# RobertKajnak/AMT-SAGA

Hardware: AMD Instinct MI355X
Metric: audio windows/sec (44.1 kHz, 2048-pt STFT) through full detect->subtract loop (higher is better)
Workload: dtype f32 (conv: split-fp16 x2 operands, f32 accumulate; 4x16 layers on the large images in the FFT domain); 1 GPU; C3: 1024 polyphonic piano windows, STFT(2048) + pitch+velocity+timing(start,end) heads + 1 subtraction iteration; windows_per_gpu=1024, n_fft=2048, hop=512, frames=516, iters=1, parallelism=windows sharded x1, event all-gather

## Files before the change

### amt-saga_amd/amt_saga/rdcnn.py

```python
import ctypes as C
import hashlib
import json
import os

import numpy as np
import torch

from . import _lib
from .device import empty, ptr, require_gpu, stream_ptr, to_dev


DEFAULT_MODE = int(os.environ.get('AMT_CONV_MODE', '3'))

_CALIBRATION_FILE = os.path.join(os.path.dirname(os.path.abspath(__file__)), 'data', 'synthetic_heads.npz')
_calibration = None


def topology_signature(cfg, seed):
    blob = json.dumps({k: cfg[k] for k in sorted(cfg)}, sort_keys=True, default=list)
    return '%s-s%d' % (hashlib.sha1(blob.encode()).hexdigest()[:10], int(seed))


def _calibration_table():
    global _calibration
# ... 204 lines not shown
        h = C.c_void_p()
        _lib.check(lib.amt_rdcnn_create(C.byref(h), C.byref(d),
                                        self._blob.ctypes.data_as(C.c_void_p), self._blob.size))
        self._net = h
        self._lib = lib
        _lib.check(lib.amt_rdcnn_set_mode(h, int(getattr(self, 'mode', DEFAULT_MODE))))

    def _release(self):
        if getattr(self, '_net', None) is not None:
            self._lib.amt_rdcnn_destroy(self._net)
        self._net = None
        self._ws = None
        if getattr(self, '_trainer', None) is not None:
            self._tlib.amt_trainer_destroy(self._trainer)
        self._trainer = None
        self._trained = False

    def __del__(self):
        try:
            self._release()
        except Exception:
            pass

    def load_weights(self, filename):
        with open(filename, 'rb') as fh:
            magic = fh.read(8)
        if magic == b'\x89HDF\r\n\x1a\n':
            from .keras_io import load_keras_weights
            self.set_weights(load_keras_weights(filename, self.layout))
            return
        with np.load(filename) as z:
            self.set_weights({k: z[k] for k in z.files})

    def save_weights(self, filename):
        self._sync_from_trainer()
        if str(filename).endswith(('.h5', '.hdf5')):
            from .keras_io import save_keras_weights
            save_keras_weights(filename, self.weights, self.cfg)
        else:
            np.savez(filename, **self.weights)

    @property
    def flops_per_window(self):
        self._ensure()
        return float(self._lib.amt_rdcnn_flops_per_window(self._net))

    @property
    def fc_pooled_layers(self):
        self._ensure()
        fn = self._lib.amt_rdcnn_fc_pooled_layers
        fn.restype, fn.argtypes = C.c_int, [C.c_void_p]
        return int(fn(self._net))

    PLAN_IMPLS = ('first_mfma', 'first_valu', 'fft_row', 'fft_packed', 'f16x3', 'bf16x6', 'f32')
    PLAN_KEYS = ('impl', 'kh', 'kw', 'cin', 'cout', 'H', 'W', 'cw', 'TH', 'TW', 'NWIN', 'masked', 'wm_ms', 'nslice', 'MT')

    def layer_plans(self, mode=None):
        self._ensure()
        fn = self._lib.amt_rdcnn_layer_plan
        fn.restype, fn.argtypes = C.c_int, [C.c_void_p, C.c_int, C.c_int, C.c_int, C.c_void_p]
        mode = self.mode if mode is None else int(mode)
        out = []
        for t in range(len(self.cfg['input_shapes'])):
            plans = []
            for i in range(self.cfg['convolutional_layer_count']):
                v = np.zeros(len(self.PLAN_KEYS), np.int32)
                _lib.check(fn(self._net, t, i, mode, v.ctypes.data_as(C.c_void_p)))
                p = dict(zip(self.PLAN_KEYS, map(int, v)), tower=t, layer=i + 1, mode=mode)
                p['impl'] = self.PLAN_IMPLS[p['impl']]
                plans.append(p)
            out.append(plans)
        return out

    def layer_outputs(self, xs):
        self._ensure()
        fn = self._lib.amt_rdcnn_layer_tap
        fn.restype, fn.argtypes = C.c_int, [C.c_void_p, C.c_int, C.c_int, C.c_void_p]
        B = xs[0].shape[0]
        acts = [[empty((B, p['H'], p['W'], p['cout'])) for p in plans] for plans in self.layer_plans()]
        try:
            for t, row in enumerate(acts):
                for i, a in enumerate(row):
                    _lib.check(fn(self._net, t, i, ptr(a)))
            y, lg = self.predict_device(xs, return_logits=True)
        finally:
            for t, row in enumerate(acts):
                for i in range(len(row)):
                    fn(self._net, t, i, None)
        return y, lg, acts

    def set_mode(self, mode):
        self.mode = int(mode)
        if self._net is not None:
            _lib.check(self._lib.amt_rdcnn_set_mode(self._net, self.mode))

    def profile(self, enable=True):
        self._ensure()
        _lib.check(self._lib.amt_rdcnn_profile(self._net, int(bool(enable))))

    def profile_read(self, reset=True):
        self._ensure()
        n = C.c_int32(0)
        _lib.check(self._lib.amt_rdcnn_profile_read(self._net, None, None, None, None, 0, C.byref(n), 0))
        cap = n.value
        desc = np.zeros((cap, 8), np.int32)
        ms = np.zeros(cap); win = np.zeros(cap); fl = np.zeros(cap)
# ... 150 lines not shown
```

### amt-saga_amd/csrc/amt_fftconv.h

```cpp
#pragma once
#include "amt_common.h"
#include "amt_launch.h"

struct amt_fftconv_layer;

struct FcEpilogue {
    const float *s1 = nullptr, *t1 = nullptr, *s2 = nullptr, *t2 = nullptr;
    const float *sc = nullptr; size_t sc_stride = 0;
    const float *sc1 = nullptr; size_t sc1_stride = 0;
    const float *sc1_w = nullptr, *sc1_s = nullptr, *sc1_t = nullptr;
    float *wmax = nullptr, *wavg = nullptr; size_t wp_stride = 0;
};

struct FcBnCopies {
    float *s1 = nullptr, *t1 = nullptr, *s2 = nullptr, *t2 = nullptr;
    hipError_t upload(const float *hs1, const float *ht1, const float *hs2, const float *ht2, int channels) {
        const float *h[4] = {hs1, ht1, hs2, ht2};
        float **d[4] = {&s1, &t1, &s2, &t2};
        hipError_t e = hipSuccess;
        for (int i = 0; i < 4 && e == hipSuccess; ++i) {
            if (h[i]) e = hipMalloc(d[i], channels * sizeof(float));
            if (h[i] && e == hipSuccess) e = hipMemcpy(*d[i], h[i], channels * sizeof(float), hipMemcpyHostToDevice);
        }
        return e;
    }
    void release() {
        for (float **p : {&s1, &t1, &s2, &t2}) { if (*p) (void)hipFree(*p); *p = nullptr; }
    }
};

int amt_fftconv_layer_create_internal(amt_fftconv_layer **out, const float *kernel);
void amt_fftconv_layer_destroy_internal(amt_fftconv_layer *L);
size_t amt_fftconv_freq_floats(int B, int H);
int amt_fftconv_forward_fft(const amt_fftconv_layer *L, const float *in_sp, size_t in_stride, int B, int H, int W,
                            float *Xf, float *amaxf, hipStream_t st);
int amt_fftconv_gemm(const amt_fftconv_layer *L, const float *Xf, const float *amaxf, int B, int H, float *Yf, hipStream_t st);
int amt_fftconv_inverse_epilogue(const amt_fftconv_layer *L, const float *Yf, const FcEpilogue &ep, int B, int H, int W,
                                 float *out_sp, size_t out_stride, float *Xf_next, float *amaxf_next, float *amax_out,
                                 hipStream_t st);

struct amt_fftpk_layer;
int amt_fftpk_layer_create_internal(amt_fftpk_layer **out, const float *kernel);
void amt_fftpk_layer_destroy_internal(amt_fftpk_layer *L);
size_t amt_fftpk_freq_floats(int B);
int amt_fftpk_forward_fft(const amt_fftpk_layer *L, const float *in_sp, size_t in_stride, int B, float *Xf, float *amaxf, hipStream_t st);
int amt_fftpk_gemm(const amt_fftpk_layer *L, const float *Xf, const float *amaxf, int B, float *Yf, hipStream_t st);
int amt_fftpk_inverse_epilogue(const amt_fftpk_layer *L, const float *Yf, const FcEpilogue &ep, int B, float *out_sp, size_t out_stride,
                               float *Xf_next, float *amaxf_next, float *amax_out, hipStream_t st);

struct FcLayer {
    amt_fftconv_layer *row = nullptr;
    amt_fftpk_layer *pk = nullptr;
    int H = 0, W = 0;
    explicit operator bool() const { return row || pk; }
};
static inline size_t fc_freq_floats(const FcLayer &l, int B) {
    return l.pk ? amt_fftpk_freq_floats(B) : amt_fftconv_freq_floats(B, l.H);
}
static inline int fc_forward_fft(const FcLayer &l, const float *in_sp, size_t in_stride, int B, float *Xf, float *amaxf, hipStream_t st) {
    return l.pk ? amt_fftpk_forward_fft(l.pk, in_sp, in_stride, B, Xf, amaxf, st)
                : amt_fftconv_forward_fft(l.row, in_sp, in_stride, B, l.H, l.W, Xf, amaxf, st);
}
static inline int fc_gemm(const FcLayer &l, const float *Xf, const float *amaxf, int B, float *Yf, hipStream_t st) {
    return l.pk ? amt_fftpk_gemm(l.pk, Xf, amaxf, B, Yf, st) : amt_fftconv_gemm(l.row, Xf, amaxf, B, l.H, Yf, st);
}
static inline int fc_inverse_epilogue(const FcLayer &l, const float *Yf, const FcEpilogue &ep, int B, float *out_sp, size_t out_stride,
                                      float *Xf_next, float *amaxf_next, float *amax_out, hipStream_t st) {
    return l.pk ? amt_fftpk_inverse_epilogue(l.pk, Yf, ep, B, out_sp, out_stride, Xf_next, amaxf_next, amax_out, st)
                : amt_fftconv_inverse_epilogue(l.row, Yf, ep, B, l.H, l.W, out_sp, out_stride, Xf_next, amaxf_next, amax_out, st);
}
```

### amt-saga_amd/csrc/amt_fftconv.hip

```cpp
#include "amt_fftconv_dev.h"
#include "amt_fftconv.h"
#include <algorithm>
#include <cmath>
#include <cstdlib>
#include <vector>

#define FC_NF 576
#define FC_NP 289
#define FC_PS 1158
#define FC_THREADS 384

struct FcRowArgs {
    const float *in_sp; size_t in_stride;
    const float *Yf;
    float *out_sp; size_t out_stride;
    float *Xf;
    float *amaxf;
    float *amax_out;
    const float *s1, *t1, *s2, *t2;
    const float *sc; size_t sc_stride;
    const float *sc1; size_t sc1_stride;
    const float *sc1_w, *sc1_s, *sc1_t;
    const float2 *tw;
    int B, H, W;
    int sf, sh;
    float *wmax, *wavg; size_t wp_stride;
};

template <bool IN_FREQ, int EPI>
__global__ __launch_bounds__(FC_THREADS, 4) void fc_row_kernel(FcRowArgs a) {
    extern __shared__ __attribute__((aligned(16))) float fc_smem[];
    const int tid = threadIdx.x;
    float *buf = fc_smem;
    float2 *tw = reinterpret_cast<float2 *>(fc_smem + 16 * FC_PS);
    const int c16 = (tid >> 2) & 15;
    const int j24 = (tid & 3) + 4 * (tid >> 6);
    const int row = blockIdx.x;
    const int b = row / a.H, h = row - b * a.H;
    for (int i = tid; i < FC_NF; i += FC_THREADS) tw[i] = a.tw[i];
    float2 x[24];
    if (IN_FREQ) {
        const int k1 = j24;
        const float *yb = a.Yf + (size_t)b * FC_NP * a.H * 64 + (size_t)h * a.sh;
        const unsigned int vlo = (unsigned)((k1 * a.sf + 2 * c16) * 4);
        const unsigned int vhi = (unsigned)(((FC_NF - k1) * a.sf + 32 + 2 * c16) * 4);
        const int kstep = 24 * a.sf;
#pragma unroll
        for (int k2 = 0; k2 < 24; ++k2) {
            if (k2 < 12) x[k2] = fc_at<float2>(yb + k2 * kstep, vlo);
            else if (k2 > 12) x[k2] = fc_at<float2>(yb - k2 * kstep, vhi);
            else x[k2] = fc_at<float2>(yb, k1 == 0 ? vlo + (unsigned)(12 * kstep * 4) : vhi - (unsigned)(12 * kstep * 4));
        }
        fc_fft24<true>(x);
        __syncthreads();
#pragma unroll
        for (int g0 = 0; g0 < 24; g0 += 8) {
            float2 w[8];
#pragma unroll
            for (int i = 0; i < 8; ++i) w[i] = tw[(g0 + i) * k1];
            __builtin_amdgcn_sched_barrier(0);
#pragma unroll
            for (int i = 0; i < 8; ++i) {
                const float2 v = fc_cmulc(x[g0 + i], w[i]);
                *reinterpret_cast<float2 *>(buf + c16 * FC_PS + ((g0 + i) * 24 + k1) * 2) = v;
            }
        }
        __syncthreads();
        const int n2 = j24;
#pragma unroll
        for (int k = 0; k < 24; ++k) x[k] = *reinterpret_cast<const float2 *>(buf + c16 * FC_PS + (n2 * 24 + k) * 2);
        fc_fft24<true>(x);
        const float inv_n = 1.0f / (float)FC_NF;
        int c0 = 2 * c16;
        if constexpr (EPI == 5) asm volatile("" : "+v"(c0));
        const float k1a = -a.s1[c0] * (inv_n * FC_LOG2E), k1b = -a.s1[c0 + 1] * (inv_n * FC_LOG2E);
        const float k0a = -a.t1[c0] * FC_LOG2E, k0b = -a.t1[c0 + 1] * FC_LOG2E;
        if constexpr (EPI == 1) {
#pragma unroll
            for (int n1 = 0; n1 < 24; ++n1) {
                float2 v;
                v.x = fc_sigmoid_affine(x[n1].x, k1a, k0a);
                v.y = fc_sigmoid_affine(x[n1].y, k1b, k0b);
                if (24 * n1 + n2 >= a.W) v = make_float2(0.f, 0.f);
                x[n1] = v;
            }
        } else {
            constexpr bool RES = EPI == 2 || EPI == 3 || EPI == 5;
            constexpr bool IDSC = EPI == 2 || EPI == 5;
            const float s2a = RES ? a.s2[c0] : 1.f, s2b = RES ? a.s2[c0 + 1] : 1.f;
            const float t2a = RES ? a.t2[c0] : 0.f, t2b = RES ? a.t2[c0 + 1] : 0.f;
            const float *scb = IDSC ? a.sc + (size_t)b * a.sc_stride + (size_t)h * a.W * 32 : nullptr;
// ... 43 lines not shown
                        v.y = (v.y + (fmaf(xi, pw1, 0.f) * ps1 + pt1)) * s2b + t2b;
                    }
                    if (w >= a.W) v = make_float2(0.f, 0.f);
                    vmax = fmaxf(vmax, fmaxf(fabsf(v.x), fabsf(v.y)));
                    if constexpr (EPI == 5) {
                        float2 m, s;
                        m.x = fmaxf(v.x, fc_quad_xor1(v.x)); m.x = fmaxf(m.x, fc_quad_xor2(m.x));
                        m.y = fmaxf(v.y, fc_quad_xor1(v.y)); m.y = fmaxf(m.y, fc_quad_xor2(m.y));
                        s.x = v.x + fc_quad_xor1(v.x); s.x = s.x + fc_quad_xor2(s.x);
                        s.y = v.y + fc_quad_xor1(v.y); s.y = s.y + fc_quad_xor2(s.y);
                        if (i == 0 || (n2e & 3) == i) { pm[batch] = m; ps[batch] = s; }
                    } else {
                        if (w < a.W) fc_at<float2>(ob, voff + (unsigned)(24 * n1 * 128)) = v;
                        x[n1] = v;
                    }
                }
                if constexpr (RES) __builtin_amdgcn_sched_barrier(0);
            }
            if (a.amax_out) {
                vmax = wave_max(vmax);
                const bool lane0 = EPI == 5 ? (n2e & 3) + 2 * c0 == 0 : (tid & 63) == 0;
                if (lane0) atomicMax(reinterpret_cast<int *>(a.amax_out) + b, __float_as_int(vmax));
            }
            if constexpr (EPI == 5) {
                __syncthreads();
                const int wv = n2e >> 2, q = n2e & 3;
                float4 *xch = reinterpret_cast<float4 *>(buf) + (wv >> 1) * 64 + (q + 2 * c0);
                if (wv & 1) {
#pragma unroll
                    for (int k = 0; k < 24 / NB; ++k) xch[k * 192] = make_float4(pm[k].x, pm[k].y, ps[k].x, ps[k].y);
                }
                __syncthreads();
                if (wv & 1) return;
                const int G = a.W >> 3;
                float *mb = a.wmax + (size_t)b * a.wp_stride + (size_t)h * G * 32;
                float *ab = a.wavg + (size_t)b * a.wp_stride + (size_t)h * G * 32;
                int cs = c0;
                asm volatile("" : "+v"(cs));
#pragma unroll
                for (int k = 0; k < 24 / NB; ++k) {
                    const float4 hi = xch[k * 192];
                    const int g = 3 * (NB * k + q) + (wv >> 1);
                    if (g < G) {
                        const unsigned int o = (unsigned)((g * 32 + cs) * 4);
                        fc_at<float2>(mb, o) = make_float2(fmaxf(pm[k].x, hi.x), fmaxf(pm[k].y, hi.y));
                        fc_at<float2>(ab, o) = make_float2((ps[k].x + hi.z) * 0.125f, (ps[k].y + hi.w) * 0.125f);
                    }
                }
                return;
            }
            if (!a.Xf) return;
        }
        __syncthreads();
    } else {
        const int n2 = j24;
        const float *rowp = a.in_sp + (size_t)b * a.in_stride + (size_t)h * a.W * 32;
#pragma unroll
        for (int n1 = 0; n1 < 24; ++n1) {
            const int w = 24 * n1 + n2;
            x[n1] = fc_at<float2>(rowp, (unsigned)((min(w, a.W - 1) * 32 + 2 * c16) * 4));
        }
#pragma unroll
        for (int n1 = 0; n1 < 24; ++n1)
            if (24 * n1 + n2 >= a.W) x[n1] = make_float2(0.f, 0.f);
        __syncthreads();
    }
    {
        int n2 = j24, cq = c16;
        asm volatile("" : "+v"(n2), "+v"(cq));
        fc_fft24<false>(x);
#pragma unroll
        for (int g0 = 0; g0 < 24; g0 += 8) {
            float2 w[8];
#pragma unroll
            for (int i = 0; i < 8; ++i) w[i] = tw[n2 * (g0 + i)];
            __builtin_amdgcn_sched_barrier(0);
#pragma unroll
            for (int i = 0; i < 8; ++i) {
                const float2 v = cmul(x[g0 + i], w[i]);
                *reinterpret_cast<float2 *>(buf + cq * FC_PS + ((g0 + i) * 24 + n2) * 2) = v;
            }
        }
        __syncthreads();
        int k1 = j24, cp = c16;
        asm volatile("" : "+v"(k1), "+v"(cp));
#pragma unroll
        for (int n = 0; n < 24; ++n) x[n] = *reinterpret_cast<const float2 *>(buf + cp * FC_PS + (k1 * 24 + n) * 2);
        fc_fft24<false>(x);
        float fmax_ = 0.f;
        float *xb = a.Xf + (size_t)b * FC_NP * a.H * 64 + (size_t)h * a.sh;
        const unsigned int vlo = (unsigned)((k1 * a.sf + 2 * cp) * 4);
        const unsigned int vhi = (unsigned)(((FC_NF - k1) * a.sf + 32 + 2 * cp) * 4);
        const int kstep = 24 * a.sf;
#pragma unroll
        for (int k2 = 0; k2 < 24; ++k2) {
            if (k2 < 12) fc_at<float2>(xb + k2 * kstep, vlo) = x[k2];
            else if (k2 > 12) fc_at<float2>(xb - k2 * kstep, vhi) = x[k2];
            else fc_at<float2>(xb, k1 == 0 ? vlo + (unsigned)(12 * kstep * 4) : vhi - (unsigned)(12 * kstep * 4)) = x[k2];
            if (k2 == 0 || k2 == 12) {
                if (k1 == 0) fc_at<float2>(xb + k2 * kstep, vlo + 128) = x[k2];
            }
            asm("v_max3_f32 %0, |%1|, |%2|, %0" : "+v"(fmax_) : "v"(x[k2].x), "v"(x[k2].y));
        }
        fmax_ = wave_max(fmax_);
        if ((tid & 63) == 0) atomicMax(reinterpret_cast<int *>(a.amaxf) + b, __float_as_int(fmax_));
    }
// ... 226 lines not shown
    if (e == hipSuccess) e = hipMemcpy(L->tw, tw.data(), tw.size() * sizeof(float2), hipMemcpyHostToDevice);
    if (e != hipSuccess) {
        snprintf(amt_hip_err_buf, sizeof(amt_hip_err_buf), "fftconv upload: %s", hipGetErrorString(e));
        amt_fftconv_layer_destroy_internal(L);
        return AMT_E_HIP;
    }
    *out = L;
    return AMT_OK;
}

void amt_fftconv_layer_destroy_internal(amt_fftconv_layer *L) {
    if (!L) return;
    for (void *p : {(void *)L->gw, (void *)L->gsw, (void *)L->tw})
        if (p) (void)hipFree(p);
    L->bn.release();
    delete L;
}

size_t amt_fftconv_freq_floats(int B, int H) { return (size_t)FC_NP * B * H * 64; }

static void fc_strides(int H, int *sf, int *sh) { *sf = H * 64; *sh = 64; }

static const size_t FC_ROW_LDS = (size_t)(16 * FC_PS) * 4 + FC_NF * sizeof(float2);
template <bool IN_FREQ, int EPI>
static int fc_row_launch_t(const FcRowArgs &a, hipStream_t st) {
    return amt_launch<fc_row_kernel<IN_FREQ, EPI>>(FC_ROW_LDS, a.B * a.H, FC_THREADS, FC_ROW_LDS, st, a);
}
template <bool IN_FREQ>
static int fc_row_launch(const FcRowArgs &a, hipStream_t st) {
    if (!IN_FREQ) return fc_row_launch_t<false, 1>(a, st);
    if (a.wmax) {
        if (!a.wavg || !a.sc || a.sc1 || a.out_sp || a.Xf || a.W < 8) return AMT_E_UNSUPPORTED;
        return fc_row_launch_t<true, 5>(a, st);
    }
    if (!a.out_sp) {
        if (a.sc || a.sc1 || a.amax_out || !a.Xf) return AMT_E_UNSUPPORTED;
        return fc_row_launch_t<true, 1>(a, st);
    }
    if (a.sc) return fc_row_launch_t<true, 2>(a, st);
    if (a.sc1) return fc_row_launch_t<true, 3>(a, st);
    return fc_row_launch_t<true, 4>(a, st);
}

int amt_fftconv_forward_fft(const amt_fftconv_layer *L, const float *in_sp, size_t in_stride, int B, int H, int W,
                            float *Xf, float *amaxf, hipStream_t st) {
    if (!L || !in_sp || !Xf || !amaxf || W + 15 > FC_NF) return AMT_E_INVALID;
    AMT_HIP_CHECK(hipMemsetAsync(amaxf, 0, (size_t)B * sizeof(float), st));
    FcRowArgs a{};
    a.in_sp = in_sp; a.in_stride = in_stride; a.Xf = Xf; a.amaxf = amaxf; a.tw = L->tw; a.B = B; a.H = H; a.W = W;
    fc_strides(H, &a.sf, &a.sh);
    return fc_row_launch<false>(a, st);
}

int amt_fftconv_gemm(const amt_fftconv_layer *L, const float *Xf, const float *amaxf, int B, int H, float *Yf, hipStream_t st) {
    if (!L || !Xf || !Yf || !amaxf) return AMT_E_INVALID;
    if (H > 20) return AMT_E_UNSUPPORTED;
    const size_t rows_cap = (size_t)FC_CW * H;
    const size_t lds = 2 * (rows_cap + 1) * FC_APITCH * sizeof(_Float16) + (size_t)4 * 16 * FC_OPITCH * 4 + 2 * FC_CW * 4 + rows_cap * 4 +
                       2 * rows_cap + 16;
    const int nchunks = (B + FC_CW - 1) / FC_CW;
    int per = 1;
    while ((size_t)((nchunks + per - 1) / per) * FC_NP > 4096 && per < 16) per *= 2;
    FcGemmArgs a{Xf, Yf, amaxf, L->gw, L->gsw, B, H, per, 0, 0};
    fc_strides(H, &a.sf, &a.sh);
    return amt_launch<fc_gemm_kernel>(lds, dim3(FC_NP, (nchunks + per - 1) / per), 256, lds, st, a);
}

int amt_fftconv_inverse_epilogue(const amt_fftconv_layer *L, const float *Yf, const FcEpilogue &ep, int B, int H, int W,
                                 float *out_sp, size_t out_stride, float *Xf_next, float *amaxf_next, float *amax_out,
                                 hipStream_t st) {
    if (!L || !Yf || !ep.s1 || !ep.t1 || (!out_sp && !Xf_next && !ep.wmax)) return AMT_E_INVALID;
    if (Xf_next && !amaxf_next) return AMT_E_INVALID;
    if (Xf_next) AMT_HIP_CHECK(hipMemsetAsync(amaxf_next, 0, (size_t)B * sizeof(float), st));
    FcRowArgs a{};
    a.Yf = Yf; a.out_sp = out_sp; a.out_stride = out_stride; a.Xf = Xf_next; a.amaxf = amaxf_next; a.amax_out = amax_out;
    a.s1 = ep.s1; a.t1 = ep.t1; a.s2 = ep.s2; a.t2 = ep.t2; a.sc = ep.sc; a.sc_stride = ep.sc_stride;
    a.sc1 = ep.sc1; a.sc1_stride = ep.sc1_stride; a.sc1_w = ep.sc1_w; a.sc1_s = ep.sc1_s; a.sc1_t = ep.sc1_t;
    a.wmax = ep.wmax; a.wavg = ep.wavg; a.wp_stride = ep.wp_stride;
    a.tw = L->tw; a.B = B; a.H = H; a.W = W;
    fc_strides(H, &a.sf, &a.sh);
    return fc_row_launch<true>(a, st);
}

extern "C" {

int amt_fftconv_create(amt_fftconv_layer **layer, const float *kernel_host, const float *s1, const float *t1,
                       const float *s2, const float *t2) {
    if (!layer || !kernel_host || !s1 || !t1) return AMT_E_INVALID;
    int rc = amt_fftconv_layer_create_internal(layer, kernel_host);
    if (rc != AMT_OK) return rc;
    if ((*layer)->bn.upload(s1, t1, s2, t2, 32) != hipSuccess) { amt_fftconv_layer_destroy_internal(*layer); *layer = nullptr; return AMT_E_HIP; }
    return AMT_OK;
}

int amt_fftconv_destroy(amt_fftconv_layer *layer) { amt_fftconv_layer_destroy_internal(layer); return AMT_OK; }

size_t amt_fftconv_workspace_bytes(int B, int H) { return (2 * amt_fftconv_freq_floats(B, H) + 2 * (size_t)B) * sizeof(float); }

int amt_fftconv_run(const amt_fftconv_layer *L, const float *in, const float *shortcut, int B, int H, int W, float *out,
                    void *workspace, size_t workspace_bytes, int repeat_gemm, void *stream) {
    if (!L || !in || !out || !workspace || B <= 0 || H <= 0 || W <= 0) return AMT_E_INVALID;
    if (W + 15 > FC_NF) return AMT_E_UNSUPPORTED;
    if (workspace_bytes < amt_fftconv_workspace_bytes(B, H)) return AMT_E_NOMEM;
    hipStream_t st = (hipStream_t)stream;
    float *Xf = (float *)workspace, *Yf = Xf + amt_fftconv_freq_floats(B, H), *amaxf = Yf + amt_fftconv_freq_floats(B, H);
    const size_t stride = (size_t)H * W * 32;
// ... 11 lines not shown
```

### amt-saga_amd/csrc/amt_rdcnn.hip

```cpp
#include "amt_common.h"
#include "amt_launch.h"
#include "amt_fftconv.h"
#include "amt_convh.h"
#include "amt_rdcnn_topology.h"
#include <vector>
#include <algorithm>
#include <cmath>
#include <cstdlib>

#include "amt_conv_f32.h"
#include "amt_conv_bf16x6.h"
#include "amt_conv_f16x3.h"
#include "amt_rdcnn_small.h"

#define RD_BN_EPS 1e-3f

struct ConvPlan {
    int TH = 0, TW = 0, NWIN = 1;
    size_t lds = 0;
    int nslice = 1, cw = 0;
    bool masked = false;
    int wm_ms = 0;
    size_t wm_lds = 0;
    double eff = 0;
    void *w = nullptr;
};
struct ConvOp {
    int cin, cout, H, W, kh, kw;
    float *s1 = nullptr, *t1 = nullptr, *s2 = nullptr, *t2 = nullptr;
    bool residual = false;
    int sc_proj = -1;
    int pool_after = 0;
    ConvPlan f32;
    int MT = 2;
    ConvPlan bf16;
    ConvPlan f16;
    int sw = 0;
    std::vector<float> k_host;
    FcLayer fc;
};
struct ProjOp {
    int cin, cout, H, W, ph, pw, HO, WO;
    float *w = nullptr, *s = nullptr, *t = nullptr;
};
struct Tower {
    int in_h, in_w, ph, pw;
    std::vector<ConvOp> convs;
    std::vector<ProjOp> projs;
    size_t max_act = 0;
    int out_h, out_w, out_c;
};
struct ProfPending { hipEvent_t e0, e1; int tower, layer, windows; };
struct ProfAcc { double ms = 0, windows = 0; long launches = 0; };
struct amt_rdcnn {
    mutable bool prof_on = false;
    mutable std::vector<ProfPending> prof_pending;
    mutable std::vector<hipEvent_t> prof_free;
    mutable std::vector<std::vector<ProfAcc>> prof_acc;
    mutable std::vector<std::vector<float *>> taps;
    amt_rdcnn_desc d;
    std::vector<Tower> towers;
    std::vector<void *> allocs;
    float *d1w = nullptr, *d1b = nullptr, *d2w = nullptr, *d2b = nullptr;
    int flat = 0;
    double flops = 0;
    mutable int mode = 0;
    bool fc_pooled = true;
};

template <class T>
static int upload(amt_rdcnn *n, const void *h, size_t bytes, T **out) {
    void *d = nullptr;
    if (hipMalloc(&d, bytes) != hipSuccess) return AMT_E_NOMEM;
    n->allocs.push_back(d);
    if (hipMemcpy(d, h, bytes, hipMemcpyHostToDevice) != hipSuccess) return AMT_E_HIP;
    *out = static_cast<T *>(d);
    return AMT_OK;
}
static int upload_folded_bn(amt_rdcnn *n, const float *bn, int c, const float *bias, float **s_out, float **t_out) {
    const float *g = bn, *b = bn + c, *m = bn + 2 * c, *v = bn + 3 * c;
    std::vector<float> s(c), t(c);
    for (int i = 0; i < c; ++i) {
        const float sc = g[i] / sqrtf(v[i] + RD_BN_EPS);
        s[i] = sc;
        t[i] = b[i] + ((bias ? bias[i] : 0.f) - m[i]) * sc;
    }
    const int rc = upload(n, s.data(), c * sizeof(float), s_out);
    return rc != AMT_OK ? rc : upload(n, t.data(), c * sizeof(float), t_out);
}

template <class F>
static void for_each_tile(int H, int W, int pcap, int max_win, F consider) {
    if (H * W <= pcap)
        for (int nw = std::min(pcap / (H * W), max_win); nw >= 1; --nw) consider(H, W, nw);
    for (int TH = 1; TH <= H && TH <= pcap; ++TH) {
        int TW = pcap / TH;
        if (TW > W) TW = W;
        if (TW >= 1) consider(TH, TW, 1);
        const int nct = (W + TW - 1) / TW;
        const int TW2 = (W + nct - 1) / nct;
        if (TW2 >= 1 && TW2 <= TW) consider(TH, TW2, 1);
    }
}

static void choose_tile(ConvOp &c) {
    ConvPlan &p = c.f32;
    double best = -1;
    for (int MT = 2; MT >= 1; --MT) {
        const int pcap = 128 * MT;
        for_each_tile(c.H, c.W, pcap, pcap, [&](int TH, int TW, int NWIN) {
            const size_t posin = (size_t)NWIN * (TH + c.kh - 1) * (TW + c.kw - 1);
            const size_t lds = posin * RD_CSTRIDE * 4 + 2 * (size_t)RD_CC * p.cw * 4 + (size_t)pcap * 8;
            if (lds > 150 * 1024) return;
            const double tiles = (double)((c.H + TH - 1) / TH) * ((c.W + TW - 1) / TW) / NWIN;
            double eff = (double)c.H * c.W / (tiles * pcap);
            if (lds > 78 * 1024) eff *= 0.93;
            if (eff > best + 1e-9) { best = eff; p.TH = TH; p.TW = TW; p.NWIN = NWIN; c.MT = MT; p.lds = lds; p.eff = eff; }
        });
    }
}
// ... 304 lines not shown
        if (!std::isfinite(kern[q])) finite = false;
        wmax = std::max(wmax, fabsf(kern[q]));
    }
    if (c.f16.TH > 0 && finite && wmax > 0.f) {
        c.sw = hx_weight_shift(wmax);
        const std::vector<unsigned short> ws = pack_f16x3(kern, ntap, C, fo, ldexpf(1.0f, c.sw));
        if ((rc = upload(n, ws.data(), ws.size() * 2, &c.f16.w)) != AMT_OK) return rc;
    }
    return AMT_OK;
}

__global__ __launch_bounds__(256) void tap_copy_kernel(const float *__restrict__ src, size_t stride, float *__restrict__ dst,
                                                       size_t n) {
    const float *s = src + (size_t)blockIdx.y * stride;
    float *o = dst + (size_t)blockIdx.y * n;
    for (size_t i = (size_t)blockIdx.x * 256 + threadIdx.x; i < n; i += (size_t)gridDim.x * 256) o[i] = s[i];
}

extern "C" {

size_t amt_rdcnn_param_count(const amt_rdcnn_desc *desc) {
    RdTopology tp;
    return desc && amt_rdcnn_topology(*desc, &tp) == AMT_OK ? tp.total : 0;
}

int amt_rdcnn_destroy(amt_rdcnn *net) {
    if (!net) return AMT_OK;
    for (const ProfPending &pp : net->prof_pending) { (void)hipEventDestroy(pp.e0); (void)hipEventDestroy(pp.e1); }
    for (hipEvent_t e : net->prof_free) (void)hipEventDestroy(e);
    for (void *p : net->allocs) (void)hipFree(p);
    for (Tower &t : net->towers)
        for (ConvOp &c : t.convs)
        {
            if (c.fc.row) amt_fftconv_layer_destroy_internal(c.fc.row);
            if (c.fc.pk) amt_fftpk_layer_destroy_internal(c.fc.pk);
        }
    delete net;
    return AMT_OK;
}

int amt_rdcnn_create(amt_rdcnn **out, const amt_rdcnn_desc *desc, const float *wh, size_t n_floats) {
    if (!out || !desc || !wh) return AMT_E_INVALID;
    const amt_rdcnn_desc &d = *desc;
    if (d.n_towers < 1 || d.n_towers > 2 || d.conv_layers < 1 || d.dense_units < 1 ||
        d.output_classes < 1)
        return AMT_E_INVALID;
    RdTopology tp;
    if (amt_rdcnn_topology(d, &tp) != AMT_OK) return AMT_E_UNSUPPORTED;
    if (tp.total != n_floats) return AMT_E_SHAPE;
    if (!tp.shortcut_ok) return AMT_E_UNSUPPORTED;
    amt_rdcnn *n = new amt_rdcnn();
    n->d = d;
    n->fc_pooled = amt_env_switch("AMT_FC_POOLED", true);
    n->flat = tp.flat;
    n->towers.resize(d.n_towers);
    for (int t = 0; t < d.n_towers; ++t) {
        Tower &tw = n->towers[t];
        tw.in_h = d.in_h[t]; tw.in_w = d.in_w[t]; tw.ph = d.pool_h[t]; tw.pw = d.pool_w[t];
        tw.max_act = (size_t)tw.in_h * tw.in_w;
        tw.out_h = tp.out_h[t]; tw.out_w = tp.out_w[t]; tw.out_c = tp.out_c[t];
    }
    int rc = AMT_OK;
#define RD_TRY(x) do { rc = (x); if (rc != AMT_OK) { amt_rdcnn_destroy(n); return rc; } } while (0)
    for (const RdLayer &l : tp.layers) {
        Tower &tw = n->towers[l.tower];
        ConvOp c;
        c.cin = l.cin; c.cout = l.cout; c.H = l.H; c.W = l.W; c.kh = l.kh; c.kw = l.kw;
        const float *kern = wh + l.kernel;
        RD_TRY(upload_folded_bn(n, wh + l.bn, l.cout, wh + l.bias, &c.s1, &c.t1));
        if (l.cin == 1) RD_TRY(upload(n, kern, (size_t)l.kh * l.kw * l.cout * sizeof(float), &c.f32.w));
        else RD_TRY(build_conv_variants(n, c, kern));
        n->flops += 2.0 * l.H * l.W * (double)l.kh * l.kw * l.cin * l.cout;
        tw.max_act = std::max(tw.max_act, (size_t)l.H * l.W * l.cout);
        c.residual = l.residual;
        if (l.residual && l.sc_bn) {
            ProjOp pr;
            pr.cin = l.sC; pr.cout = l.cout; pr.H = l.sH; pr.W = l.sW;
            pr.ph = l.sc_ph; pr.pw = l.sc_pw; pr.HO = l.H; pr.WO = l.W;
            RD_TRY(upload_folded_bn(n, wh + l.sc_bnorm, l.cout, l.sc_proj ? wh + l.sc_bias : nullptr, &pr.s, &pr.t));
            if (l.sc_proj) RD_TRY(upload(n, wh + l.sc_kernel, (size_t)l.sC * l.cout * sizeof(float), &pr.w));
            n->flops += 2.0 * l.H * l.W * (double)l.sC * l.cout;
            c.sc_proj = (int)tw.projs.size();
            tw.projs.push_back(pr);
        }
        if (l.residual) RD_TRY(upload_folded_bn(n, wh + l.res_bn, l.cout, nullptr, &c.s2, &c.t2));
        c.pool_after = l.pool_after ? 1 : 0;
        tw.convs.push_back(c);
    }
    RD_TRY(upload(n, wh + tp.d1_kernel, (size_t)tp.flat * d.dense_units * sizeof(float), &n->d1w));
    RD_TRY(upload(n, wh + tp.d1_bias, (size_t)d.dense_units * sizeof(float), &n->d1b));
    RD_TRY(upload(n, wh + tp.d2_kernel, (size_t)d.dense_units * d.output_classes * sizeof(float), &n->d2w));
    RD_TRY(upload(n, wh + tp.d2_bias, (size_t)d.output_classes * sizeof(float), &n->d2b));
    n->flops += 2.0 * tp.flat * d.dense_units + 2.0 * d.dense_units * d.output_classes;
#undef RD_TRY
    *out = n;
    return AMT_OK;
}

double amt_rdcnn_flops_per_window(const amt_rdcnn *net) { return net ? net->flops : 0.0; }

int amt_rdcnn_set_mode(amt_rdcnn *net, int mode) {
    if (!net || mode < 0 || mode > 3) return AMT_E_INVALID;
    if (mode == 3) {
        for (Tower &t : net->towers)
            for (ConvOp &c : t.convs)
                if (!c.fc && !c.k_host.empty()) {
// ... 127 lines not shown
        for (const ConvOp &c : t.convs)
            if (impl_is_fft(conv_impl(c, n->mode))) freq = std::max(freq, fc_freq_floats(c.fc, Bc));
    l.Yf = l.Xf + freq;
    l.amaxf = l.Yf + freq;
    if (freq) l.total += 2 * freq + (size_t)Bc + 8;
    return l;
}

size_t amt_rdcnn_workspace_bytes(const amt_rdcnn *net, int B) {
    if (!net || B <= 0) return 0;
    return ws_layout(net, std::min(B, RD_CHUNK)).total * sizeof(float);
}

static int grid_for(size_t total) {
    size_t g = (total + 255) / 256;
    return (int)std::min<size_t>(g, 65536);
}
static int launch_absmax(const float *x, size_t n, size_t stride, int B, float *amax, hipStream_t st) {
    absmax_kernel<<<dim3((unsigned)std::min<size_t>((n + 1023) / 1024, 64), B), 256, 0, st>>>(x, n, stride, amax);
    AMT_LAUNCH_CHECK();
    return AMT_OK;
}

static int prof_begin(const amt_rdcnn *net, ProfPending &pp, hipStream_t st) {
    if (!net->prof_on) return AMT_OK;
    for (hipEvent_t *pe : {&pp.e0, &pp.e1}) {
        if (!net->prof_free.empty()) { *pe = net->prof_free.back(); net->prof_free.pop_back(); }
        else AMT_HIP_CHECK(hipEventCreate(pe));
    }
    AMT_HIP_CHECK(hipEventRecord(pp.e0, st));
    return AMT_OK;
}
static int prof_end(const amt_rdcnn *net, const ProfPending &pp, hipStream_t st) {
    if (!net->prof_on) return AMT_OK;
    AMT_HIP_CHECK(hipEventRecord(pp.e1, st));
    net->prof_pending.push_back(pp);
    return AMT_OK;
}

struct FcBufs { float *Xf, *Yf, *amaxf; };
static bool fc_wpooled_ok(const amt_rdcnn *net, const Tower &tw, int i, ConvImpl impl, int H, int W) {
    const ConvOp &c = tw.convs[i];
    if (!net->fc_pooled || !impl_is_fft(impl) || !c.pool_after || tw.pw != 8 || W < 8) return false;
    if (!c.residual || (c.sc_proj >= 0 && shortcut_is_rank1(impl, c, tw.projs[c.sc_proj]))) return false;
    for (size_t j = (size_t)i + 1; j < tw.convs.size(); ++j) {
        const ConvOp &r = tw.convs[j];
        if (!r.residual) continue;
        if (r.sc_proj < 0) return false;
        const ProjOp &pr = tw.projs[r.sc_proj];
        return pr.H == H && pr.W == W && pr.cin == c.cout && pr.pw == 8 && pr.WO == W / 8;
    }
    return true;
}
static int run_fc(const ConvOp &c, const float *in, size_t in_stride, bool have_xf, int Bc, const FcEpilogue &ep,
                  const FcBufs &f, float *o, size_t o_stride, bool next_fc, float *amax_o, hipStream_t st) {
    int rc = AMT_OK;
    if (!have_xf) rc = fc_forward_fft(c.fc, in, in_stride, Bc, f.Xf, f.amaxf, st);
    if (rc == AMT_OK) rc = fc_gemm(c.fc, f.Xf, f.amaxf, Bc, f.Yf, st);
    if (rc != AMT_OK) return rc;
    const bool need_sp = !ep.wmax && (!next_fc || c.residual);
    return fc_inverse_epilogue(c.fc, f.Yf, ep, Bc, need_sp ? o : nullptr, o_stride, next_fc ? f.Xf : nullptr, f.amaxf,
                               next_fc ? nullptr : amax_o, st);
}

int amt_rdcnn_forward(const amt_rdcnn *net, const float *const *x, int B, float *y, float *logits,
                      void *workspace, size_t workspace_bytes, void *stream) {
    if (!net || !x || !y || !workspace || B <= 0) return AMT_E_INVALID;
    const amt_rdcnn_desc &d = net->d;
    for (int t = 0; t < d.n_towers; ++t) if (!x[t]) return AMT_E_INVALID;
    if (workspace_bytes < amt_rdcnn_workspace_bytes(net, B)) return AMT_E_NOMEM;
    hipStream_t st = (hipStream_t)stream;
    const int K = d.output_classes, DU = d.dense_units, flat = net->flat, mode = net->mode;
#define RD_TRY(x) do { const int rc_ = (x); if (rc_ != AMT_OK) return rc_; } while (0)

    for (int b0 = 0; b0 < B; b0 += RD_CHUNK) {
        const int Bc = std::min(RD_CHUNK, B - b0);
        float *ws = static_cast<float *>(workspace);
        const WsLayout lay = ws_layout(net, Bc, workspace);
        float *buf[4];
        for (int i = 0; i < 4; ++i) buf[i] = ws + lay.buf[i];
        float *flatbuf = ws + lay.flat, *d1 = ws + lay.dense, *lg = ws + lay.logits;
        auto amax_row = [&](int i) { return ws + lay.amax + (size_t)i * Bc; };
        const FcBufs fcb{ws + lay.Xf, ws + lay.Yf, ws + lay.amaxf};
        int flat_off = 0;
        for (int t = 0; t < d.n_towers; ++t) {
            const Tower &tw = net->towers[t];
            const float *cur = x[t] + (size_t)b0 * tw.in_h * tw.in_w;
            size_t cur_stride = (size_t)tw.in_h * tw.in_w;
            if (mode >= 2) {
                AMT_HIP_CHECK(hipMemsetAsync(amax_row(0), 0, (size_t)(d.conv_layers + 1) * Bc * sizeof(float), st));
                RD_TRY(launch_absmax(cur, cur_stride, cur_stride, Bc, amax_row(0), st));
            }
            const float *p0 = cur; size_t p0_stride = cur_stride;
            bool p0_wpooled = false;
            int H = tw.in_h, W = tw.in_w;
            const int L = (int)tw.convs.size();
            bool xf_valid = false;
            auto pick = [&](const float *a, const float *b_, const float *c_) -> float * {
                for (int i = 0; i < 4; ++i)
                    if (buf[i] != a && buf[i] != b_ && buf[i] != c_) return buf[i];
                return nullptr;
            };
            for (int i = 0; i < L; ++i) {
                const ConvOp &c = tw.convs[i];
                const ConvImpl impl = conv_impl(c, mode);
                const bool last_op = (i == L - 1) && !c.pool_after;
                float *o = last_op ? flatbuf + flat_off : pick(cur, p0, nullptr);
                const size_t o_stride = last_op ? (size_t)flat : (size_t)H * W * c.cout;
                const float *sc = nullptr; size_t sc_stride = 0;
                const ProjOp *rank1 = nullptr;
                if (c.residual && c.sc_proj >= 0) {
                    const ProjOp &pr = tw.projs[c.sc_proj];
                    if (shortcut_is_rank1(impl, c, pr)) {
                        rank1 = &pr;
                    } else {
                        float *sb = pick(cur, p0, o);
                        ProjParams pp{p0, p0_stride, sb, (size_t)pr.HO * pr.WO * pr.cout, pr.w, pr.s, pr.t,
                                      Bc, pr.H, pr.W, pr.cin, pr.cout, pr.ph, pr.pw, pr.HO, pr.WO};
                        if (p0_wpooled) { pp.W = pr.W / 8; pp.PW = 1; }
                        proj_kernel<<<dim3((pr.WO + PJ_TW - 1) / PJ_TW, pr.HO, Bc), 256,
                                      (size_t)PJ_TW * pr.cin * sizeof(float), st>>>(pp);
                        sc = sb; sc_stride = (size_t)pr.HO * pr.WO * pr.cout;
                    }
                } else if (c.residual) {
                    sc = p0; sc_stride = p0_stride;
                }
                const float *s2 = c.residual ? c.s2 : nullptr, *t2 = c.residual ? c.t2 : nullptr;
                float *amax_o = mode >= 2 ? amax_row(i + 1) : nullptr;
                const bool wpooled = fc_wpooled_ok(net, tw, i, impl, H, W);
                const size_t wp_stride = (size_t)H * (W / 8) * c.cout;
                const bool next_fc = impl_is_fft(impl) && i + 1 < L && !c.pool_after && conv_impl(tw.convs[i + 1], mode) == impl;
                float *const tap = net->taps.empty() ? nullptr : net->taps[t][i];
                if (tap && impl_is_fft(impl) && (wpooled || (next_fc && !c.residual))) return AMT_E_UNSUPPORTED;
                ProfPending prof{nullptr, nullptr, t, i, Bc};
                RD_TRY(prof_begin(net, prof, st));
                switch (impl) {
                case IMPL_FIRST_MFMA:
                    RD_TRY(launch_conv1_mfma(c, Conv1Params{cur, cur_stride, o, o_stride, sc, sc_stride, static_cast<const float *>(c.f32.w),
                                                            c.s1, c.t1, s2, t2, Bc, H, W, c.kh, c.kw, c.cout, amax_o}, st));
                    break;
                case IMPL_FIRST_VALU:
                    RD_TRY(launch_conv1(c, Conv1Params{cur, cur_stride, o, o_stride, sc, sc_stride, static_cast<const float *>(c.f32.w),
                                                       c.s1, c.t1, s2, t2, Bc, H, W, c.kh, c.kw, c.cout}, st));
                    break;
                case IMPL_FFT_ROW:
                case IMPL_FFT_PACKED: {
                    FcEpilogue ep;
                    ep.s1 = c.s1; ep.t1 = c.t1; ep.s2 = s2; ep.t2 = t2;
                    if (rank1) { ep.sc1 = p0; ep.sc1_stride = p0_stride; ep.sc1_w = rank1->w; ep.sc1_s = rank1->s; ep.sc1_t = rank1->t; }
                    else { ep.sc = sc; ep.sc_stride = sc_stride; }
                    if (wpooled) { ep.wavg = o; ep.wmax = o + (size_t)Bc * wp_stride; ep.wp_stride = wp_stride; }
                    RD_TRY(run_fc(c, cur, cur_stride, xf_valid, Bc, ep, fcb, o, o_stride, next_fc, amax_o, st));
                    xf_valid = next_fc;
                    break;
                }
                default: {
                    ConvParams cp{cur, cur_stride, o, o_stride, sc, sc_stride, static_cast<const float *>(c.f32.w), c.s1, c.t1, s2, t2,
                                  Bc, H, W, 0, 0, 1, 0, 0, c.cout};
                    if (rank1) {
                        cp.sc1 = p0; cp.sc1_win_stride = p0_stride;
                        cp.sc1_w = rank1->w; cp.sc1_s = rank1->s; cp.sc1_t = rank1->t;
                    }
                    RD_TRY(impl == IMPL_F16X3    ? launch_convh(c, cp, amax_row(i), amax_o, st)
                           : impl == IMPL_BF16X6 ? launch_conv16(c, cp, st) : launch_conv(c, cp, st));
                }
                }
                if (amax_o && !impl_writes_amax(impl) && i + 1 < L)
                    RD_TRY(launch_absmax(o, (size_t)H * W * c.cout, o_stride, Bc, amax_o, st));
                RD_TRY(prof_end(net, prof, st));
                if (tap) {
                    const size_t n = (size_t)H * W * c.cout;
                    tap_copy_kernel<<<dim3((unsigned)std::min<size_t>((n + 255) / 256, 64), Bc), 256, 0, st>>>(
                        o, o_stride, tap + (size_t)b0 * n, n);
                    AMT_LAUNCH_CHECK();
                }
                if (c.residual) { p0 = o; p0_stride = wpooled ? wp_stride : o_stride; p0_wpooled = wpooled; }
                cur = o; cur_stride = o_stride;
                if (wpooled) { cur = o + (size_t)Bc * wp_stride; cur_stride = wp_stride; }
                if (c.pool_after) {
                    const int HO = H / tw.ph, WO = W / tw.pw;
                    const bool last = (i == L - 1);
                    float *po = last ? flatbuf + flat_off : pick(cur, p0, nullptr);
                    const size_t po_stride = last ? (size_t)flat : (size_t)HO * WO * c.cout;
                    maxpool_kernel<<<grid_for((size_t)Bc * HO * WO * c.cout / 4), 256, 0, st>>>(
                        cur, cur_stride, po, po_stride, Bc, H, wpooled ? W / 8 : W, c.cout, tw.ph, wpooled ? 1 : tw.pw, HO, WO);
                    cur = po; cur_stride = po_stride; H = HO; W = WO;
                }
            }
            flat_off += tw.out_h * tw.out_w * tw.out_c;
        }
// ... 115 lines not shown
```

Measured before the change: 13960 windows/s.

## Fuse first 4x16 conv into FFT-row forward transform of second layer

Adds a CONV1 path to the FFT row kernel that computes the 1->32 channel 4x16 first convolution with MFMA plus BN+sigmoid directly in shared memory, then feeds the result straight into the forward row FFT. This avoids writing the 32-channel first-layer activation to global memory and reading it back for the FFT, and drops one kernel launch per tower. It is enabled by default under mode 3 when the tower shape matches, and can be turned off with an env switch. The cost is more per-block work and register pressure in the FFT kernel, and the fused path must reproduce the original conv numerics.

```diff
diff --git a/amt-saga_amd/amt_saga/rdcnn.py b/amt-saga_amd/amt_saga/rdcnn.py
--- a/amt-saga_amd/amt_saga/rdcnn.py
+++ b/amt-saga_amd/amt_saga/rdcnn.py
@@ -280,6 +280,23 @@
         fn.restype, fn.argtypes = C.c_int, [C.c_void_p]
         return int(fn(self._net))
 
+    @property
+    def fc_conv1_towers(self):
+        self._ensure()
+        fn = self._lib.amt_rdcnn_fc_conv1_towers
+        fn.restype, fn.argtypes = C.c_int, [C.c_void_p]
+        return int(fn(self._net))
+
+    def first_transform(self, x, tower=0):
+        self._ensure()
+        fn = self._lib.amt_rdcnn_first_transform
+        fn.restype = C.c_int
+        fn.argtypes = [C.c_void_p, C.c_int, C.c_void_p, C.c_int, C.c_void_p, C.c_void_p, C.c_void_p, C.c_void_p]
+        B, H, W = x.shape
+        act, xf, amaxf = empty((B, H, W, 32)), empty((B, 289, H, 64)), empty((B,))
+        _lib.check(fn(self._net, int(tower), ptr(x), B, ptr(act), ptr(xf), ptr(amaxf), stream_ptr()))
+        return xf, amaxf
+
     PLAN_IMPLS = ('first_mfma', 'first_valu', 'fft_row', 'fft_packed', 'f16x3', 'bf16x6', 'f32')
     PLAN_KEYS = ('impl', 'kh', 'kw', 'cin', 'cout', 'H', 'W', 'cw', 'TH', 'TW', 'NWIN', 'masked', 'wm_ms', 'nslice', 'MT')
 
diff --git a/amt-saga_amd/csrc/amt_fftconv.h b/amt-saga_amd/csrc/amt_fftconv.h
--- a/amt-saga_amd/csrc/amt_fftconv.h
+++ b/amt-saga_amd/csrc/amt_fftconv.h
@@ -34,6 +34,8 @@
 size_t amt_fftconv_freq_floats(int B, int H);
 int amt_fftconv_forward_fft(const amt_fftconv_layer *L, const float *in_sp, size_t in_stride, int B, int H, int W,
                             float *Xf, float *amaxf, hipStream_t st);
+int amt_fftconv_forward_fft_conv1(const amt_fftconv_layer *L, const float *in1, size_t in1_stride, const float *w1, const float *s1,
+                                  const float *t1, int B, int H, int W, float *Xf, float *amaxf, hipStream_t st);
 int amt_fftconv_gemm(const amt_fftconv_layer *L, const float *Xf, const float *amaxf, int B, int H, float *Yf, hipStream_t st);
 int amt_fftconv_inverse_epilogue(const amt_fftconv_layer *L, const float *Yf, const FcEpilogue &ep, int B, int H, int W,
                                  float *out_sp, size_t out_stride, float *Xf_next, float *amaxf_next, float *amax_out,
diff --git a/amt-saga_amd/csrc/amt_fftconv.hip b/amt-saga_amd/csrc/amt_fftconv.hip
--- a/amt-saga_amd/csrc/amt_fftconv.hip
+++ b/amt-saga_amd/csrc/amt_fftconv.hip
@@ -9,6 +9,9 @@
 #define FC_NP 289
 #define FC_PS 1158
 #define FC_THREADS 384
+
+typedef float fc_f32x16 __attribute__((ext_vector_type(16)));
+__device__ __forceinline__ float fc_sigmoid_div(float v) { return 1.0f / (1.0f + __expf(-v)); }
 
 struct FcRowArgs {
     const float *in_sp; size_t in_stride;
@@ -25,6 +28,8 @@
     int B, H, W;
     int sf, sh;
     float *wmax, *wavg; size_t wp_stride;
+    const float *c1_in; size_t c1_stride;
+    const float *c1_w;
 };
 
 template <bool IN_FREQ, int EPI>
@@ -37,6 +42,7 @@
     const int j24 = (tid & 3) + 4 * (tid >> 6);
     const int row = blockIdx.x;
     const int b = row / a.H, h = row - b * a.H;
+    constexpr bool CONV1 = !IN_FREQ && EPI == 6;
     for (int i = tid; i < FC_NF; i += FC_THREADS) tw[i] = a.tw[i];
     float2 x[24];
     if (IN_FREQ) {
@@ -186,6 +192,71 @@
             if (!a.Xf) return;
         }
         __syncthreads();
+    } else if constexpr (CONV1) {
+        float *xin = buf;
+        const int RP = a.W + 15;
+        const int half = (tid >> 5) & 1, co = tid & 31;
+        const int wv = __builtin_amdgcn_readfirstlane(tid >> 6);
+        const int ntiles = (a.W + 31) >> 5;
+        const float *img = a.c1_in + (size_t)b * a.c1_stride;
+        {
+            float v[6];
+#pragma unroll
+            for (int u = 0; u < 6; ++u) {
+                const int i = tid + FC_THREADS * u;
+                const int r = (i >= RP ? 1 : 0) + (i >= 2 * RP ? 1 : 0) + (i >= 3 * RP ? 1 : 0), ci = i - r * RP;
+                const int gr = h + r - 1, gc = ci - 7;
+                const bool in = gr >= 0 && gr < a.H && gc >= 0 && gc < a.W;
+                v[u] = img[in ? gr * a.W + gc : 0];
+                if (!in) v[u] = 0.f;
+            }
+#pragma unroll
+            for (int u = 0; u < 6; ++u)
+                if (tid + FC_THREADS * u < 4 * RP) xin[tid + FC_THREADS * u] = v[u];
+        }
+        float bq[32];
+#pragma unroll
+        for (int i = 0; i < 32; ++i) bq[i] = a.c1_w[(2 * i + half) * 32 + co];
+        const float s1 = a.s1[co], t1 = a.t1[co];
+        fc_f32x16 acc[3];
+        __syncthreads();
+#pragma unroll
+        for (int s = 0; s < 3; ++s) {
+            if (wv + 6 * s >= ntiles) continue;
+            const int pos = 32 * (wv + 6 * s) + co;
+            const int ab = (pos < a.W ? pos : 0) + half;
+#pragma unroll
+            for (int e = 0; e < 16; ++e) acc[s][e] = 0.f;
+#pragma unroll
+            for (int i = 0; i < 32; ++i) {
+                const float av = xin[ab + (i >> 3) * RP + 2 * (i & 7)];
+                acc[s] = __builtin_amdgcn_mfma_f32_32x32x2f32(av, bq[i], acc[s], 0, 0, 0);
+            }
+#pragma unroll
+            for (int e = 0; e < 16; ++e) acc[s][e] = fc_sigmoid_div(acc[s][e] * s1 + t1);
+        }
+        __syncthreads();
+#pragma unroll
+        for (int s = 0; s < 3; ++s) {
+            if (wv + 6 * s >= ntiles) continue;
+#pragma unroll
+            for (int e = 0; e < 16; ++e) {
+                const int pos = 32 * (wv + 6 * s) + (e & 3) + 8 * (e >> 2) + 4 * half;
+                if (pos < a.W) buf[(co >> 1) * FC_PS + 2 * pos + (co & 1)] = acc[s][e];
+            }
+        }
+        __syncthreads();
+        int n2 = j24, cq = c16;
+        asm volatile("" : "+v"(n2), "+v"(cq));
+#pragma unroll
+        for (int n1 = 0; n1 < 24; ++n1) {
+            const int w = 24 * n1 + n2;
+            x[n1] = *reinterpret_cast<const float2 *>(buf + cq * FC_PS + 2 * min(w, a.W - 1));
+        }
+#pragma unroll
+        for (int n1 = 0; n1 < 24; ++n1)
+            if (24 * n1 + n2 >= a.W) x[n1] = make_float2(0.f, 0.f);
+        __syncthreads();
     } else {
         const int n2 = j24;
         const float *rowp = a.in_sp + (size_t)b * a.in_stride + (size_t)h * a.W * 32;
@@ -518,6 +589,17 @@
     return fc_row_launch<false>(a, st);
 }
 
+int amt_fftconv_forward_fft_conv1(const amt_fftconv_layer *L, const float *in1, size_t in1_stride, const float *w1, const float *s1,
+                                  const float *t1, int B, int H, int W, float *Xf, float *amaxf, hipStream_t st) {
+    if (!L || !in1 || !w1 || !s1 || !t1 || !Xf || !amaxf || W < 1 || W + 15 > FC_NF) return AMT_E_INVALID;
+    AMT_HIP_CHECK(hipMemsetAsync(amaxf, 0, (size_t)B * sizeof(float), st));
+    FcRowArgs a{};
+    a.c1_in = in1; a.c1_stride = in1_stride; a.c1_w = w1; a.s1 = s1; a.t1 = t1;
+    a.Xf = Xf; a.amaxf = amaxf; a.tw = L->tw; a.B = B; a.H = H; a.W = W;
+    fc_strides(H, &a.sf, &a.sh);
+    return fc_row_launch_t<false, 6>(a, st);
+}
+
 int amt_fftconv_gemm(const amt_fftconv_layer *L, const float *Xf, const float *amaxf, int B, int H, float *Yf, hipStream_t st) {
     if (!L || !Xf || !Yf || !amaxf) return AMT_E_INVALID;
     if (H > 20) return AMT_E_UNSUPPORTED;
diff --git a/amt-saga_amd/csrc/amt_rdcnn.hip b/amt-saga_amd/csrc/amt_rdcnn.hip
--- a/amt-saga_amd/csrc/amt_rdcnn.hip
+++ b/amt-saga_amd/csrc/amt_rdcnn.hip
@@ -66,6 +66,7 @@
     double flops = 0;
     mutable int mode = 0;
     bool fc_pooled = true;
+    bool fc_conv1 = true;
 };
 
 template <class T>
@@ -476,6 +477,7 @@
     amt_rdcnn *n = new amt_rdcnn();
     n->d = d;
     n->fc_pooled = amt_env_switch("AMT_FC_POOLED", true);
+    n->fc_conv1 = amt_env_switch("AMT_FC_CONV1", true);
     n->flat = tp.flat;
     n->towers.resize(d.n_towers);
     for (int t = 0; t < d.n_towers; ++t) {
@@ -709,6 +711,47 @@
     }
     return true;
 }
+static bool fc_conv1_fused_rule(bool enabled, int mode, int cin, int cout, int kh, int kw, bool next_fft_row, bool spatial_reader) {
+    return enabled && mode == 3 && cin == 1 && cout == 32 && kh == 4 && kw == 16 && next_fft_row && !spatial_reader;
+}
+static bool fc_conv1_fused_ok(const amt_rdcnn *net, int t, int mode) {
+    const Tower &tw = net->towers[t];
+    if (tw.convs.size() < 2) return false;
+    const ConvOp &c = tw.convs[0];
+    const bool tapped = !net->taps.empty() && net->taps[t][0];
+    return fc_conv1_fused_rule(net->fc_conv1, mode, c.cin, c.cout, c.kh, c.kw, conv_impl(tw.convs[1], mode) == IMPL_FFT_ROW,
+                               c.residual || c.pool_after || tapped);
+}
+static int launch_conv1_fused(const Tower &tw, const float *in, size_t in_stride, int Bc, const FcBufs &f, hipStream_t st) {
+    const ConvOp &c = tw.convs[0];
+    return amt_fftconv_forward_fft_conv1(tw.convs[1].fc.row, in, in_stride, static_cast<const float *>(c.f32.w), c.s1, c.t1, Bc, c.H, c.W,
+                                         f.Xf, f.amaxf, st);
+}
+int amt_rdcnn_fc_conv1_rule(int enabled, int mode, int cin, int cout, int kh, int kw, int next_fft_row, int spatial_reader) {
+    return fc_conv1_fused_rule(enabled != 0, mode, cin, cout, kh, kw, next_fft_row != 0, spatial_reader != 0) ? 1 : 0;
+}
+int amt_rdcnn_fc_conv1_towers(const amt_rdcnn *net) {
+    if (!net) return AMT_E_INVALID;
+    int n = 0;
+    for (size_t t = 0; t < net->towers.size(); ++t) n += fc_conv1_fused_ok(net, (int)t, net->mode) ? 1 : 0;
+    return n;
+}
+int amt_rdcnn_first_transform(const amt_rdcnn *net, int tower, const float *x, int B, float *act, float *Xf, float *amaxf, void *stream) {
+    if (!net || tower < 0 || tower >= (int)net->towers.size() || !x || !act || !Xf || !amaxf || B <= 0) return AMT_E_INVALID;
+    const Tower &tw = net->towers[tower];
+    if (tw.convs.size() < 2 || conv_impl(tw.convs[0], net->mode) != IMPL_FIRST_MFMA || tw.convs[0].pool_after ||
+        tw.convs[0].residual || conv_impl(tw.convs[1], net->mode) != IMPL_FFT_ROW)
+        return AMT_E_UNSUPPORTED;
+    hipStream_t st = (hipStream_t)stream;
+    const ConvOp &c = tw.convs[0];
+    const size_t in_stride = (size_t)c.H * c.W, act_stride = in_stride * c.cout;
+    const FcBufs f{Xf, nullptr, amaxf};
+    if (fc_conv1_fused_ok(net, tower, net->mode)) return launch_conv1_fused(tw, x, in_stride, B, f, st);
+    const int rc = launch_conv1_mfma(c, Conv1Params{x, in_stride, act, act_stride, nullptr, 0, static_cast<const float *>(c.f32.w),
+                                                    c.s1, c.t1, nullptr, nullptr, B, c.H, c.W, c.kh, c.kw, c.cout, nullptr}, st);
+    return rc != AMT_OK ? rc : fc_forward_fft(tw.convs[1].fc, act, act_stride, B, Xf, amaxf, st);
+}
+
 static int run_fc(const ConvOp &c, const float *in, size_t in_stride, bool have_xf, int Bc, const FcEpilogue &ep,
                   const FcBufs &f, float *o, size_t o_stride, bool next_fc, float *amax_o, hipStream_t st) {
     int rc = AMT_OK;
@@ -793,6 +836,11 @@
                 RD_TRY(prof_begin(net, prof, st));
                 switch (impl) {
                 case IMPL_FIRST_MFMA:
+                    if (i == 0 && fc_conv1_fused_ok(net, t, mode)) {
+                        RD_TRY(launch_conv1_fused(tw, cur, cur_stride, Bc, fcb, st));
+                        xf_valid = true;
+                        break;
+                    }
                     RD_TRY(launch_conv1_mfma(c, Conv1Params{cur, cur_stride, o, o_stride, sc, sc_stride, static_cast<const float *>(c.f32.w),
                                                             c.s1, c.t1, s2, t2, Bc, H, W, c.kh, c.kw, c.cout, amax_o}, st));
                     break;
```

Result: no change. 14080 windows/s, median of 6 (+0.9%).
